# refresh-bio/LZ-ANI

Hardware: AMD Instinct MI355X
Metric: genome-pairs/sec + achieved HBM GB/s, 10k×40kbp all2all at 1/2/4/8 GPUs (higher is better)
Workload: dtype u32 (2-bit packed symbols, 64-bit lane masks; f64 only in the anchor/seed arbitration)

## Files before the change

### lz-ani_amd/csrc/lzani_kernels_pairs.h

```cpp
#pragma once

namespace lzani {

enum { SEED_BM_BITS = 14, SEED_BM_WORDS = 1 << (SEED_BM_BITS - 5), NQUEUES = 8 };
enum { AQ_CAP = 64, AQ_MAXCHUNKS = 32, AQ_LANE_CAP = 32, AQ_LDS_CAND = 128,
       SEED_PAD = 96,
       SEED_LDS_WORDS = SEED_BM_WORDS + SEED_PAD };
static_assert(2 * AQ_LDS_CAND <= SEED_BM_WORDS, "the candidate buffers of refill live in the seed bitmap");
enum : u32 { AQ_COMPLEX = 0x80000000u, AQ_LONG = 0x40000000u, AQ_POS = 0x3FFFFFFFu };
enum { AQ_NONE = 0x7FFFFFFF };

__device__ __forceinline__ u64 wballot(bool b) { return __builtin_amdgcn_ballot_w64(b); }
__device__ __forceinline__ u32 rep4(u32 b) { return __builtin_amdgcn_perm(b, b, 0u); }

#if defined(LZANI_RTC)
#define LZ_RTC_PARAMS Params{LZANI_P_MAL, LZANI_P_MSL, LZANI_P_MRD, LZANI_P_MQD, LZANI_P_REG, LZANI_P_AW, LZANI_P_AM, LZANI_P_AR}
#else
#define LZ_RTC_PARAMS Params{11, 7, 40, 40, 35, 15, 7, 3}
#endif
LZ_HD constexpr Params folded_params(int defp)
{
    return defp == 2 ? Params{15, 9, 40, 40, 60, 15, 7, 3} : defp == 9 ? LZ_RTC_PARAMS : Params{11, 7, 40, 40, 35, 15, 7, 3};
}
LZ_HD constexpr bool chain_params_ok(const Params& p)
// ... 740 lines not shown
            "ds_or_b32 %[a0], %[t]\n\t" \
            WORD("a1", "bq", K1) \
            "ds_or_b32 %[a1], %[bq]\n\t" \
            WORD("aq", "t", QK) \
            "ds_read_b32 %[aq], %[aq]\n\t" \
            "ds_write_b32 %[a0], %[zero]\n\t" \
            "ds_write_b32 %[a1], %[zero]\n\t" \
            "s_waitcnt lgkmcnt(2)\n\t" \
            "v_and_b32_e32 %[aq], %[aq], %[t]\n\t" \
            "v_cmp_ne_u32_e64 %[seed], 0, %[aq]\n\t"
#define LZ_NC_ROUND_F(WORD) LZ_NC_ROUND_X(WORD, "s_waitcnt vmcnt(0)", "qk", "rk0", "rk1")
#define LZ_NC_FTURN(WORDF, P, N, IC, IN, RN, CQ, C0, C1, NQ, N0, N1, SFX) \
            "Lnc_fturn" SFX "_%=:\n\t" \
            "s_bitcmp0_b32 %[" P "], 15\n\t" \
            "s_cbranch_scc1 Lnc_fnogo" SFX "_%=\n\t" \
            "s_bfe_u32 %[qh], %[" P "], 0x70008\n\t"         \
            "v_readlane_b32 %[" N "], %[alen], %[qh]\n\t"    \
            "v_readlane_b32 %[ap], %[apos], %[qh]\n\t" \
            "v_readlane_b32 %[bpos], %[aref], %[qh]\n\t" \
            "s_bfe_u32 %[t0], %[" N "], 0x80011\n\t" \
            "s_sub_i32 %[gap], %[ap], %[" IC "]\n\t" \
            "s_add_i32 %[" IN "], %[ap], %[t0]\n\t" \
            "s_add_i32 %[" RN "], %[bpos], %[t0]\n\t" \
            LZ_NC_LOADS_X(IN, RN, NQ, N0, N1) \
            LZ_NC_ROUND_X(WORDF, "s_waitcnt vmcnt(3)", CQ, C0, C1) \
            LZ_NC_SEEDS \
            "s_cbranch_scc1 Lnc_frec" SFX "_%=\n\t"          \
            "s_mov_b32 %[t2], %[qh]\n\t" \
            LZ_NC_COUNT
#define LZ_NC_FIX \
            "s_bfm_b64 %[m2], %[NT], 0\n\t" \
            "s_and_b64 %[seed], %[seed], %[m2]\n\t" \
            "v_cmp_gt_u32_e64 %[m2], %[NR1], %[lane]\n\t" \
            "v_cmp_gt_u32_e32 vcc, %[NT], %[lane]\n\t" \
            "s_nop 1\n\t" \
            "v_cndmask_b32_e64 %[rk1], -1, %[rk1], %[m2]\n\t" \
            "v_cndmask_b32_e32 %[qk], -1, %[qk], vcc\n\t" \
            "v_cmp_ne_u32_e32 vcc, -1, %[qk]\n\t"           \
            "s_and_b64 %[seed], %[seed], vcc\n\t" \
            "s_and_b64 %[m], %[m], vcc\n"
#define LZ_NC_SEEDS \
            "s_add_i32 %[t0], %[gap], 1\n\t" \
            "s_min_u32 %[t0], %[t0], %[NT]\n\t" \
            "s_bfm_b64 %[m], %[t0], 0\n\t" \
            "s_and_b64 %[m], %[m], %[seed]\n\t" LZ_NC_NOSEED
#define LZ_NC_COMMIT \
            "s_sub_i32 %[plit], %[t1], %[kb]\n\t"            \
            "s_sub_i32 %[prs], %[ap], %[kb]\n\t"             \
            "s_bfe_u32 %[t0], %[rec], 0x50018\n\t"           \
            "s_bfe_u32 %[lastlit], %[rec], 0x40014\n\t"      \
            "s_add_i32 %[t2], %[blen], %[t0]\n\t" \
            "s_sub_i32 %[lastb], %[t2], %[lastlit]\n\t"      \
            "s_add_i32 %[lastb], %[lastb], %[kc]\n\t" \
            "s_add_i32 %[lastlit], %[lastlit], %[kb]\n\t"    \
            "s_sub_i32 %[lastlit], %[lastlit], %[kc]\n\t" \
            "s_add_i32 %[i], %[ap], %[t2]\n\t" \
            "s_add_i32 %[rend], %[bpos], %[t2]\n\t" \
            "s_mov_b32 %[pre], %[i]\n\t" \
            "s_add_i32 %[qh], %[qh], 1\n\t" \
            LZ_NC_COUNT
        int gap, cls, fok;
        u64 m2;
        const u32* const rt2 = uniform_ptr(reinterpret_cast<const u32*>(R.t2));
        const u32* const qt2 = uniform_ptr(reinterpret_cast<const u32*>(Q.t2));
        const int qend = __builtin_amdgcn_readfirstlane((R.nfree && Q.nfree) ? iend : -(1 << 30));
        const int ocl_u = __builtin_amdgcn_readfirstlane(open_cl), oclit_u = __builtin_amdgcn_readfirstlane(open_clit);
#ifdef LZANI_CHAIN_PRIO
#define LZ_NC_PRIO_ON "s_setprio 2\n\t"
#define LZ_NC_PRIO_OFF "s_setprio 0\n\t"
#else
#define LZ_NC_PRIO_ON
#define LZ_NC_PRIO_OFF
#endif
#define LZ_NC_SPLITCHK \
            "v_readlane_b32 %[t0], %[apos], %[qh]\n\t" \
            "s_cmp_gt_i32 %[t0], %[ilim]\n\t" \
            "s_cbranch_scc1 Lnc_end_%=\n\t"
#define LZ_NC_SPLITGEN \
            "s_cmp_lg_u32 %[tnt], 0\n\t" \
            "s_cbranch_scc1 Lnc_chk_%=\n\t"
#define LZ_NC_SPLITIN , [tnt] "s"(tnt_u)
#define LZ_NC_ASM(WORD, WORDF) LZ_NC_ASM_X(WORD, WORDF, "", "", )
#define LZ_NC_ASM_X(WORD, WORDF, SPLCHK, SPLGEN, SPLIN) \
        asm volatile( \
            LZ_NC_PRIO_ON \
            "s_mov_b32 %[code], 0\n\t" \
            "s_mov_b32 %[lastb], 0\n\t" \
            "s_mov_b32 %[lastlit], 0\n\t" \
            "s_mov_b32 %[atm], 0\n\t" \
            "s_mov_b32 %[atl], 0\n\t" \
            "s_mov_b32 %[atc], 0\n\t" \
            "s_mov_b64 %[m2], -1\n\t"                       \
             \
             \
            "v_add_u32_e32 %[w1], 64, %[lane]\n\t" \
            "v_subrev_u32_e32 %[dumv], %[WIN], %[w1]\n\t" \
            "v_min_u32_e32 %[w1], %[w1], %[dumv]\n\t" \
            "v_add_u32_e32 %[dumv], %[wdum], %[lane]\n\t"   \
            "s_nop 3\n" \
            "Lnc_top_%=:\n\t" \
             \
            "s_cmp_ge_i32 %[qh], %[qc]\n\t" \
            "s_cbranch_scc1 Lnc_end_%=\n\t" \
            "v_readlane_b32 %[t0], %[apos], %[qh]\n\t" \
            "s_cmp_ge_i32 %[t0], %[i]\n\t" \
            "s_cbranch_scc1 Lnc_nodrop_%=\n\t" \
            "v_cmp_le_i32_e32 vcc, %[qh], %[lane]\n\t" \
            "v_cmp_le_i32_e64 %[m], %[i], %[apos]\n\t" \
            "s_and_b64 %[m], %[m], vcc\n\t" \
            "s_ff1_i32_b64 %[qh], %[m]\n\t" \
            "s_min_u32 %[qh], %[qh], 64\n\t" \
            "s_cmp_ge_i32 %[qh], %[qc]\n\t" \
            "s_cbranch_scc1 Lnc_end_%=\n" \
            "Lnc_nodrop_%=:\n\t" \
            "s_cmp_gt_i32 %[i], %[ilim]\n\t" \
            "s_cbranch_scc1 Lnc_end_%=\n\t" \
            "s_cmp_gt_i32 %[rend], %[rlim]\n\t" \
            "s_cbranch_scc1 Lnc_end_%=\n\t" \
            SPLCHK \
            LZ_NC_LOADS_F \
             \
             \
            "v_readlane_b32 %[blen], %[alen], %[qh]\n\t" \
            "v_readlane_b32 %[ap], %[apos], %[qh]\n\t" \
            "v_readlane_b32 %[bpos], %[aref], %[qh]\n\t" \
            "v_readlane_b32 %[rec], %[aext], %[qh]\n\t" \
            "s_mov_b32 %[t2], 0\n\t" \
            "s_mov_b32 %[cls], 0\n\t"                         \
            "s_bfe_u32 %[code], %[blen], 0x10010\n\t"        \
            "s_sext_i32_i8 %[blen], %[blen]\n\t"             \
            "s_sub_i32 %[gap], %[ap], %[i]\n\t" \
            "s_cmp_lt_i32 %[blen], 1\n\t" \
            "s_cbranch_scc1 Lnc_chk_%=\n\t" \
            "s_cmp_le_i32 %[gap], %[MQD]\n\t" \
            "s_cbranch_scc1 Lnc_close_%=\n" \
            "Lnc_distant_%=:\n\t" \
            "s_cmp_lt_i32 %[prs], 0\n\t" \
            "s_cbranch_scc1 Lnc_kept_%=\n\t" \
            "s_sub_i32 %[t1], %[pre], %[prs]\n\t" \
            "s_cmp_ge_i32 %[t1], %[REG]\n\t" \
            "s_cbranch_scc1 Lnc_kept_%=\n\t" \
            "s_sub_i32 %[t1], %[ap], %[prs]\n\t" \
            "s_add_i32 %[t1], %[t1], %[plit]\n"              \
            "Lnc_avail_%=:\n\t" \
             \
             \
            "s_cmp_eq_u32 %[code], 0\n\t" \
            "s_cbranch_scc1 Lnc_gen_%=\n\t" \
            "s_cmp_lt_i32 %[t1], %[AW]\n\t" \
            "s_cbranch_scc1 Lnc_gen_%=\n\t" \
            "s_and_b32 %[kb], %[rec], 15\n\t" \
            "s_bfe_u32 %[kc], %[rec], 0x40004\n\t" \
            "s_mov_b32 %[fok], 1\n\t" \
            "s_branch Lnc_ok_%=\n" \
            "Lnc_gen_%=:\n\t" \
            SPLGEN \
            "s_bitcmp0_b32 %[rec], 29\n\t"                   \
            "s_cbranch_scc1 Lnc_chk_%=\n\t" \
            "s_min_i32 %[t0], %[t1], %[ap]\n\t" \
            "s_min_i32 %[t0], %[t0], %[bpos]\n\t"            \
            "s_mov_b32 %[kb], 0\n\t"                           \
            "s_mov_b32 %[kc], 0\n\t" \
            "s_mov_b32 %[fok], 0\n\t" \
            "s_cmp_lt_i32 %[t0], 1\n\t" \
            "s_cbranch_scc1 Lnc_ok_%=\n\t" \
            "s_bitcmp1_b32 %[rec], 30\n\t" \
            "s_cbranch_scc1 Lnc_brkb_%=\n\t" \
            "s_min_i32 %[code], %[t0], %[AW]\n\t"            \
            "s_bfm_b32 %[code], %[code], 0\n\t"              \
            "s_and_b32 %[code], %[code], %[rec]\n\t" \
            "s_cbranch_scc1 Lnc_chk_%=\n\t" \
            "s_cmp_le_i32 %[t0], %[AW]\n\t" \
            "s_cbranch_scc1 Lnc_ok_%=\n\t" \
            "s_branch Lnc_chk_%=\n" \
            "Lnc_brkb_%=:\n\t"                                \
            "s_cmp_lt_i32 %[t0], %[AW]\n\t"                  \
            "s_cbranch_scc1 Lnc_chk_%=\n\t" \
            "s_and_b32 %[kb], %[rec], 15\n\t" \
            "s_bfe_u32 %[kc], %[rec], 0x40004\n\t" \
            "s_mov_b32 %[fok], 1\n"                           \
            "Lnc_ok_%=:\n\t" \
            "s_mov_b32 %[t2], 1\n" \
            "Lnc_chk_%=:\n\t" \
            LZ_NC_ROUND_F(WORD) \
            "s_mov_b32 %[code], 1\n\t" \
            LZ_NC_SEEDS \
            "s_cbranch_scc1 Lnc_sseed_%=\n"                  \
            "Lnc_noseed_%=:\n\t" \
            "s_cmp_lt_i32 %[blen], 1\n\t" \
            "s_cbranch_scc1 Lnc_npl_%=\n\t"                  \
            "s_mov_b32 %[code], 2\n\t" \
            "s_cmp_eq_u32 %[t2], 0\n\t" \
            "s_cbranch_scc1 Lnc_end_%=\n\t"                  \
            "s_cmp_eq_u32 %[cls], 0\n\t" \
            "s_cbranch_scc1 Lnc_commit_%=\n\t" \
             \
             \
             \
            "s_cmp_lg_u32 %[lastb], 0\n\t" \
            "s_cselect_b32 %[t0], %[lastb], %[ocl]\n\t" \
            "s_cselect_b32 %[t2], %[lastlit], %[oclit]\n\t" \
            "s_cmp_eq_u32 %[t0], 0\n\t" \
            "s_cbranch_scc1 Lnc_commit_%=\n\t" \
            "s_add_i32 %[t2], %[t2], %[t0]\n\t" \
            "s_cmp_lt_i32 %[t2], %[REG]\n\t" \
            "s_cbranch_scc1 Lnc_commit_%=\n\t" \
            "s_sub_i32 %[t2], %[t2], %[t0]\n\t" \
            "s_add_i32 %[atm], %[atm], %[t0]\n\t" \
            "s_add_i32 %[atl], %[atl], %[t2]\n\t" \
            "s_add_i32 %[atc], %[atc], 1\n" \
            "Lnc_commit_%=:\n\t" \
            LZ_NC_COMMIT \
            "s_mov_b32 %[code], 0\n\t" \
            "s_cmp_eq_u32 %[fok], 0\n\t" \
            "s_cbranch_scc1 Lnc_top_%=\n" \
             \
             \
             \
            "Lnc_fast_%=:\n\t" \
             \
             \
             \
             \
            "s_sub_i32 %[fok], %[prs], %[plit]\n\t" \
            "s_sub_i32 %[t2], %[qh], 1\n\t"                 \
            "v_readlane_b32 %[cls], %[alen], %[t2]\n"       \
            "Lnc_fstart_%=:\n\t" \
            LZ_NC_LOADS_F \
             \
             \
             \
             \
             \
            LZ_NC_FTURN(WORDF, "cls", "blen", "i", "t1", "kb", "qk", "rk0", "rk1", "qkb", "rk0b", "rk1b", "") \
            LZ_NC_FTURN(WORDF, "blen", "cls", "t1", "i", "rend", "qkb", "rk0b", "rk1b", "qk", "rk0", "rk1", "2") \
            "s_branch Lnc_fturn_%=\n" \
            "Lnc_fnogo2_%=:\n\t" \
            "s_mov_b32 %[i], %[t1]\n\t" \
            "s_mov_b32 %[rend], %[kb]\n\t" \
            "s_mov_b32 %[cls], %[blen]\n\t" \
            "s_branch Lnc_fnogo_%=\n" \
            "Lnc_frec2_%=:\n\t" \
            "s_mov_b32 %[i], %[t1]\n\t" \
            "s_mov_b32 %[rend], %[kb]\n\t" \
            "s_mov_b32 %[t0], %[cls]\n\t" \
            "s_mov_b32 %[cls], %[blen]\n\t" \
            "s_mov_b32 %[blen], %[t0]\n\t" \
            "s_waitcnt vmcnt(0)\n\t"                         \
            "v_mov_b32_e32 %[qk], %[qkb]\n\t" \
            "v_mov_b32_e32 %[rk0], %[rk0b]\n\t" \
            "v_mov_b32_e32 %[rk1], %[rk1b]\n\t" \
            "s_branch Lnc_frec_%=\n" \
             \
            "Lnc_fcont_%=:\n\t" \
            "s_bfe_u32 %[t0], %[blen], 0x80011\n\t" \
            "s_add_i32 %[i], %[ap], %[t0]\n\t" \
            "s_add_i32 %[rend], %[bpos], %[t0]\n\t" \
            "s_mov_b32 %[t2], %[qh]\n\t" \
            "s_mov_b32 %[cls], %[blen]\n\t" \
            LZ_NC_COUNT \
            "s_branch Lnc_fstart_%=\n" \
            "Lnc_fnogo_%=:\n\t"                             \
            "s_add_i32 %[qh], %[t2], 1\n" \
             \
            "Lnc_frec_%=:\n\t" \
            "v_readlane_b32 %[t0], %[apos], %[t2]\n\t" \
            "v_readlane_b32 %[t1], %[alen], %[t2]\n\t" \
            "v_readlane_b32 %[kc], %[aext], %[t2]\n\t" \
            "s_sext_i32_i8 %[t1], %[t1]\n\t" \
            "s_and_b32 %[kb], %[kc], 15\n\t" \
            "s_sub_i32 %[prs], %[t0], %[kb]\n\t" \
            "s_sub_i32 %[plit], %[t0], %[fok]\n\t" \
            "s_sub_i32 %[plit], %[plit], %[kb]\n\t" \
            "s_bfe_u32 %[lastlit], %[kc], 0x40014\n\t" \
            "s_bfe_u32 %[t0], %[kc], 0x50018\n\t" \
            "s_add_i32 %[t1], %[t1], %[t0]\n\t" \
            "s_sub_i32 %[lastb], %[t1], %[lastlit]\n\t" \
            "s_bfe_u32 %[t0], %[kc], 0x40004\n\t" \
            "s_add_i32 %[lastb], %[lastb], %[t0]\n\t" \
            "s_add_i32 %[lastlit], %[lastlit], %[kb]\n\t" \
            "s_sub_i32 %[lastlit], %[lastlit], %[t0]\n\t" \
            "s_mov_b32 %[pre], %[i]\n\t" \
            "s_bitcmp0_b32 %[cls], 15\n\t" \
            "s_cbranch_scc1 Lnc_top_%=\n"                    \
            "Lnc_fseed_%=:\n\t"                              \
            "s_mov_b32 %[code], 1\n\t" \
            LZ_NC_FIX \
            "s_cmp_eq_u64 %[m], 0\n\t"                       \
            "s_cbranch_scc1 Lnc_snone_%=\n" \
             \
             \
             \
             \
             \
             \
            "Lnc_seedev_%=:\n\t" \
            "s_ff1_i32_b64 %[t0], %[m]\n"                    \
            "Lnc_sdl_%=:\n\t" \
            "v_readlane_b32 %[t1], %[qk], %[t0]\n\t"         \
            "s_add_i32 %[t2], %[t0], %[MRD]\n\t"             \
            "s_sub_i32 %[kc], %[t2], 64\n\t" \
            "s_max_i32 %[kc], %[kc], 0\n\t" \
            "s_min_u32 %[kb], %[t2], 64\n\t" \
            "s_sub_i32 %[kb], 64, %[kb]\n\t"                 \
            "v_cmp_eq_u32_e32 vcc, %[t1], %[rk1]\n\t" \
            "s_bfm_b64 %[m2], %[kc], 0\n\t" \
            "s_and_b64 %[m2], %[m2], vcc\n\t" \
            "v_cmp_eq_u32_e32 vcc, %[t1], %[rk0]\n\t" \
            "s_bcnt1_i32_b64 %[kc], %[m2]\n\t" \
            "s_lshl_b64 vcc, vcc, %[kb]\n\t" \
            "s_bcnt1_i32_b64 %[t1], vcc\n\t" \
            "s_add_i32 %[t2], %[t1], %[kc]\n\t" \
            LZ_NC_WHY(2) \
            "s_cmp_eq_u32 %[t2], 0\n\t" \
            "s_cbranch_scc1 Lnc_sfalse_%=\n\t"               \
            "s_cmp_lg_u32 %[t2], 1\n\t" \
            "s_cbranch_scc1 Lnc_end_%=\n\t"                  \
            "s_ff1_i32_b64 %[t2], vcc\n\t" \
            "s_sub_i32 %[t2], %[t2], %[kb]\n\t" \
            "s_ff1_i32_b64 %[kc], %[m2]\n\t" \
            "s_add_i32 %[kc], %[kc], 64\n\t" \
            "s_cmp_lg_u32 %[t1], 0\n\t" \
            "s_cselect_b32 %[t2], %[t2], %[kc]\n\t"          \
            "s_add_i32 %[rec], %[rend], %[t2]\n\t"           \
            "s_add_i32 %[cls], %[i], %[t0]\n\t"              \
             \
             \
             \
             \
            LZ_NC_WHY(1) \
            "s_cmp_lg_u32 %[t0], %[gap]\n\t" \
            "s_cbranch_scc1 Lnc_snoq_%=\n\t" \
            "s_cmp_lt_i32 %[blen], 1\n\t" \
            "s_cbranch_scc1 Lnc_end_%=\n\t" \
            "s_cmp_lg_u32 %[bpos], %[rec]\n\t" \
            "s_cbranch_scc1 Lnc_end_%=\n" \
            "Lnc_snoq_%=:\n\t" \
             \
             \
             \
            "s_sub_i32 %[t1], %[qend], %[CQ64]\n\t" \
            LZ_NC_WHY(3) \
            "s_cmp_gt_i32 %[cls], %[t1]\n\t" \
            "s_cbranch_scc1 Lnc_end_%=\n\t" \
            "s_sub_i32 %[t1], %[rlim], %[C41M]\n\t" \
            "s_lshr_b32 %[t1], %[t1], 1\n\t" \
// ... 101 lines not shown
            "v_lshlrev_b32_e32 %[t], 1, %[t]\n\t" \
            "v_lshlrev_b32_e32 %[bq], 1, %[bq]\n\t" \
            "v_and_b32_e32 %[t], 30, %[t]\n\t" \
            "v_and_b32_e32 %[bq], 30, %[bq]\n\t" \
            "v_lshrrev_b32_e32 %[rk0], %[t], %[rk0]\n\t" \
            "v_lshrrev_b32_e32 %[rk1], %[bq], %[rk1]\n\t" \
            "v_xor_b32_e32 %[rk0], %[rk0], %[rk1]\n\t" \
            "v_and_b32_e32 %[rk0], 3, %[rk0]\n\t" \
            "v_cmp_eq_u32_e64 %[m], 0, %[rk0]\n\t" \
             \
            "v_add_u32_e32 %[t], %[gap], %[lane]\n\t" \
            "v_add_u32_e32 %[bq], %[kc], %[lane]\n\t" \
            "v_lshlrev_b32_e32 %[t], 1, %[t]\n\t" \
            "v_lshlrev_b32_e32 %[bq], 1, %[bq]\n\t" \
            "v_and_b32_e32 %[t], 30, %[t]\n\t" \
            "v_and_b32_e32 %[bq], 30, %[bq]\n\t" \
            "v_lshrrev_b32_e32 %[qk], %[t], %[qk]\n\t" \
            "v_lshrrev_b32_e32 %[a0], %[bq], %[a0]\n\t" \
            "v_xor_b32_e32 %[qk], %[qk], %[a0]\n\t" \
            "v_and_b32_e32 %[qk], 3, %[qk]\n\t" \
            "v_cmp_eq_u32_e64 %[m2], 0, %[qk]\n\t" \
             \
            "v_add_u32_e32 %[t], %[fok], %[lane]\n\t" \
            "v_add_u32_e32 %[bq], %[t1], %[lane]\n\t" \
            "v_lshlrev_b32_e32 %[t], 1, %[t]\n\t" \
            "v_lshlrev_b32_e32 %[bq], 1, %[bq]\n\t" \
            "v_and_b32_e32 %[t], 30, %[t]\n\t" \
            "v_and_b32_e32 %[bq], 30, %[bq]\n\t" \
            "v_lshrrev_b32_e32 %[a1], %[t], %[a1]\n\t" \
            "v_lshrrev_b32_e32 %[aq], %[bq], %[aq]\n\t" \
            "v_xor_b32_e32 %[a1], %[a1], %[aq]\n\t" \
            "v_and_b32_e32 %[a1], 3, %[a1]\n\t" \
            "v_cmp_ne_u32_e32 vcc, 0, %[a1]\n\t" \
            "s_and_b64 %[m], %[m], %[seed]\n\t"              \
            "s_and_b64 %[m2], %[m2], %[seed]\n\t"            \
            "s_mov_b64 %[seed], vcc\n\t"                     \
             \
            "s_bcnt1_i32_b64 %[t2], %[m2]\n\t" \
            "s_mov_b64 vcc, %[m]\n\t" \
            "s_nop 0\n\t" \
            "v_mbcnt_lo_u32_b32 %[t], vcc_lo, 0\n\t" \
            "v_mbcnt_hi_u32_b32 %[t], vcc_hi, %[t]\n\t" \
            "s_mov_b64 vcc, %[m2]\n\t" \
            "s_nop 0\n\t" \
            "v_mbcnt_lo_u32_b32 %[bq], vcc_lo, 0\n\t" \
            "v_mbcnt_hi_u32_b32 %[bq], vcc_hi, %[bq]\n\t" \
            "v_add_u32_e32 %[t], %[t2], %[t]\n\t" \
            "v_sub_u32_e32 %[t], %[t], %[bq]\n\t" \
            "v_cmp_ge_u32_e32 vcc, %[kb], %[lane]\n\t" \
            "s_nop 1\n\t" \
            "v_cndmask_b32_e32 %[t], 0, %[t], vcc\n\t"       \
            "s_nop 1\n\t" \
            "v_max_u32_dpp %[t], %[t], %[t] row_shr:1 row_mask:0xf bank_mask:0xf bound_ctrl:0\n\t" \
            "s_nop 1\n\t" \
            "v_max_u32_dpp %[t], %[t], %[t] row_shr:2 row_mask:0xf bank_mask:0xf bound_ctrl:0\n\t" \
            "s_nop 1\n\t" \
            "v_max_u32_dpp %[t], %[t], %[t] row_shr:4 row_mask:0xf bank_mask:0xf bound_ctrl:0\n\t" \
            "s_nop 1\n\t" \
            "v_max_u32_dpp %[t], %[t], %[t] row_shr:8 row_mask:0xf bank_mask:0xf bound_ctrl:0\n\t" \
            "s_nop 1\n\t" \
            "v_max_u32_dpp %[t], %[t], %[t] row_bcast:15 row_mask:0xa bank_mask:0xf\n\t" \
            "s_nop 1\n\t" \
            "v_max_u32_dpp %[t], %[t], %[t] row_bcast:31 row_mask:0xc bank_mask:0xf\n\t" \
            "s_nop 1\n\t" \
            "v_readlane_b32 %[t2], %[t], 63\n\t"             \
             \
             \
             \
            "s_mov_b64 vcc, %[seed]\n\t" \
            "s_lshl_b32 %[gap], vcc_lo, %[AW1]\n\t" \
            "s_lshr_b32 %[kb], vcc_lo, %[AW1C]\n\t" \
            "s_lshl_b32 %[kc], vcc_hi, %[AW1]\n\t" \
            "s_or_b32 %[kc], %[kc], %[kb]\n\t" \
            "s_lshr_b32 %[kb], vcc_hi, %[AW1C]\n\t" \
            "v_mov_b32_e32 %[rk0], %[gap]\n\t" \
            "v_mov_b32_e32 %[rk1], %[kc]\n\t" \
            "v_mov_b32_e32 %[qk], %[kb]\n\t" \
            "v_cmp_gt_u32_e32 vcc, 32, %[lane]\n\t" \
            "v_alignbit_b32 %[a0], %[rk1], %[rk0], %[lane]\n\t" \
            "v_alignbit_b32 %[a1], %[qk], %[rk1], %[lane]\n\t" \
            "v_cndmask_b32_e32 %[a0], %[a1], %[a0], vcc\n\t" \
            "v_and_b32_e32 %[a0], %[AWM], %[a0]\n\t" \
            "v_bcnt_u32_b32 %[a1], %[a0], 0\n\t" \
            "v_and_b32_e32 %[a0], %[ARM], %[a0]\n\t" \
            "v_cmp_lt_u32_e32 vcc, %[AM], %[a1]\n\t"             \
            "v_cmp_eq_u32_e64 %[m], 0, %[a0]\n\t"            \
            "s_nop 0\n\t" \
            "s_cmp_eq_u64 vcc, 0\n\t" \
            "s_cbranch_scc1 Lnc_end_%=\n\t"                  \
            "s_ff1_i32_b64 %[kb], vcc\n\t" \
            "s_cmp_ge_u32 %[kb], 63\n\t" \
            "s_cbranch_scc1 Lnc_end_%=\n\t" \
            "s_add_i32 %[kb], %[kb], 1\n\t" \
            "s_bfm_b64 %[m2], %[kb], 0\n\t" \
            "s_and_b64 %[m], %[m], %[m2]\n\t"                \
            "s_mov_b32 %[kb], 0\n\t"                          \
            "s_mov_b32 %[kc], 0\n\t"                          \
            "s_cbranch_scc0 Lnc_sext_%=\n\t" \
            "s_flbit_i32_b64 %[kb], %[m]\n\t" \
            "s_sub_i32 %[kb], 64, %[kb]\n\t"                 \
            "s_bfm_b64 %[m2], %[kb], 0\n\t" \
            "s_and_b64 %[m2], %[m2], %[seed]\n\t" \
            "s_bcnt1_i32_b64 %[kc], %[m2]\n"                  \
            "Lnc_sext_%=:\n\t" \
             \
            "s_cmp_lg_u32 %[lastb], 0\n\t" \
            "s_cselect_b32 %[gap], %[lastb], %[ocl]\n\t" \
            "s_cselect_b32 %[rec], %[lastlit], %[oclit]\n\t" \
            "s_add_i32 %[gap], %[gap], %[t2]\n\t"            \
            "s_add_i32 %[gap], %[gap], %[blen]\n\t" \
            "s_add_i32 %[gap], %[gap], %[kb]\n\t" \
            "s_sub_i32 %[lastb], %[gap], %[kc]\n\t"          \
            "s_add_i32 %[rec], %[rec], %[t0]\n\t" \
            "s_sub_i32 %[rec], %[rec], %[t2]\n\t" \
            "s_add_i32 %[lastlit], %[rec], %[kc]\n\t"        \
            "s_add_i32 %[i], %[t1], %[kb]\n\t" \
            "s_add_i32 %[rend], %[fok], %[kb]\n\t" \
            "s_mov_b32 %[pre], %[i]\n\t" \
            "s_mov_b32 %[code], 0\n\t" \
            "s_mov_b64 %[m2], -1\n\t" \
            LZ_NC_COUNT \
            "s_branch Lnc_top_%=\n" \
             \
             \
            "Lnc_sfalse_%=:\n\t" \
            "s_bitset0_b64 %[m], %[t0]\n\t" \
            "s_cmp_eq_u64 %[m], 0\n\t" \
            "s_cbranch_scc1 Lnc_snone_%=\n\t" \
            "s_ff1_i32_b64 %[t0], %[m]\n\t" \
            "s_branch Lnc_sdl_%=\n" \
            "Lnc_snone_%=:\n\t" \
            "s_mov_b32 %[code], 0\n\t" \
            "s_mov_b64 %[m2], -1\n\t" \
            "s_bitcmp1_b32 %[cls], 15\n\t" \
            "s_cbranch_scc1 Lnc_fcont_%=\n\t" \
            "s_mov_b64 %[m2], 0\n\t" \
            "s_branch Lnc_top_%=\n" \
            "Lnc_sseed_%=:\n\t"                             \
            "s_cmp_eq_u64 %[m2], 0\n\t" \
            "s_mov_b64 %[m2], -1\n\t" \
            "s_cbranch_scc1 Lnc_noseed_%=\n\t" \
            "s_branch Lnc_fseed_%=\n" \
            "Lnc_kept_%=:\n\t"                               \
            "s_mov_b32 %[cls], 1\n\t"                         \
            "s_mov_b32 %[t1], %[gap]\n\t" \
            "s_branch Lnc_avail_%=\n" \
            "Lnc_close_%=:\n\t"                              \
            "s_add_i32 %[t1], %[rend], %[gap]\n\t" \
            "s_sub_i32 %[t1], %[bpos], %[t1]\n\t" \
            "s_abs_i32 %[t1], %[t1]\n\t" \
            "s_cmp_le_i32 %[t1], %[MRD]\n\t" \
            "s_cbranch_scc1 Lnc_chk_%=\n\t" \
            "s_branch Lnc_distant_%=\n" \
            "Lnc_npl_%=:\n\t" \
            LZ_NC_FIX \
            "Lnc_end_%=:\n\t" \
            "s_waitcnt vmcnt(0) lgkmcnt(0)\n\t" \
            LZ_NC_PRIO_OFF \
            "s_nop 4" \
            : LZ_NC_COUNT_OPERAND [i] "+s"(i), [rend] "+s"(r_end), [qh] "+s"(qh), [prs] "+s"(prev_rs), [pre] "+s"(prev_re), [plit] "+s"(pre_lit), \
              [code] "=&s"(code), [ap] "=&s"(ap), [bpos] "=&s"(bpos), [blen] "=&s"(blen), [lastb] "=&s"(last_cl), [lastlit] "=&s"(last_clit), [rec] "=&s"(rec), \
              [t0] "=&s"(t0), [t1] "=&s"(t1), [t2] "=&s"(t2), [kb] "=&s"(kb), [kc] "=&s"(kc), [m] "=&s"(m), [seed] "=&s"(seed), \
              [gap] "=&s"(gap), [cls] "=&s"(cls), [fok] "=&s"(fok), [atm] "=&s"(add_tm), [atl] "=&s"(add_tl), [atc] "=&s"(add_tc), [m2] "=&s"(m2), \
              [rk0] "=&v"(rk0), [rk1] "=&v"(rk1), [qk] "=&v"(qk), [a0] "=&v"(a0), [a1] "=&v"(a1), [aq] "=&v"(aq), [t] "=&v"(t), [bq] "=&v"(bq), [w1] "=&v"(w1), [dumv] "=&v"(dumv), [qkb] "=&v"(qkb), [rk0b] "=&v"(rk0b), [rk1b] "=&v"(rk1b) \
            : [qc] "s"(qc_u), [ilim] "s"(ilim_u), [rlim] "s"(rlim_u), [qks] "s"(qks), [rks] "s"(rks), [ocl] "s"(ocl_u), [oclit] "s"(oclit_u), \
              [rt2] "s"(rt2), [qt2] "s"(qt2), [qend] "s"(qend), [wdum] "s"((int)SEED_BM_WORDS) SPLIN, \
              [apos] "v"(a_pos), [alen] "v"(a_len), [aref] "v"(a_ref), [aext] "v"(a_ext), [lane] "v"(lane), \
              [ldsb] "v"(ldsb), [zero] "v"(zero), [one] "v"(one), \
              [MQD] "n"(MQD), [MRD] "n"(MRD), [REG] "n"(REG), [AW] "n"(AW), [NT] "n"(NT), [WIN] "s"((int)WIN), [NR1] "n"(WIN - 64), [MSL] "n"(MSL), [MSL64] "n"(MSL + 64), [C41M] "n"(3 * MRD + 1 - WIN - MSL), [C40M] "n"(MRD - MSL), [CQ64] "n"(MRD + 64), [C2MRD] "n"(2 * MRD), \
              [AW1] "n"(AW - 1), [AW1C] "n"(33 - AW), [AWM] "n"((1 << AW) - 1), [ARM] "n"(((1 << AR) - 1) << (AW - AR)), [AM] "n"(AM), [KS5] "n"(2 * MSL + 5), [KS] "n"(2 * MSL) \
            : "vcc", "scc", "memory");
#ifdef LZANI_PHASE_TIME
        const unsigned long long pt_t0 = pt_now();
#endif
        if constexpr (SPLITW) {
            if constexpr (MSL == 9) { LZ_NC_ASM_X(LZ_NC_WORD9, LZ_NC_WORD9, LZ_NC_SPLITCHK, LZ_NC_SPLITGEN, LZ_NC_SPLITIN) }
            else if constexpr (MSL == 8) { LZ_NC_ASM_X(LZ_NC_WORD8, LZ_NC_WORD8, LZ_NC_SPLITCHK, LZ_NC_SPLITGEN, LZ_NC_SPLITIN) }
            else if constexpr (CP::NF) { LZ_NC_ASM_X(LZ_NC_WORD7, LZ_NC_WORD7N, LZ_NC_SPLITCHK, LZ_NC_SPLITGEN, LZ_NC_SPLITIN) }
            else { LZ_NC_ASM_X(LZ_NC_WORD7, LZ_NC_WORD7, LZ_NC_SPLITCHK, LZ_NC_SPLITGEN, LZ_NC_SPLITIN) }
        } else
        if constexpr (MSL == 9) { LZ_NC_ASM(LZ_NC_WORD9, LZ_NC_WORD9) }
        else if constexpr (MSL == 8) { LZ_NC_ASM(LZ_NC_WORD8, LZ_NC_WORD8) }
        else if constexpr (CP::NF) { LZ_NC_ASM(LZ_NC_WORD7, LZ_NC_WORD7N) }
        else { LZ_NC_ASM(LZ_NC_WORD7, LZ_NC_WORD7) }
#ifdef LZANI_PHASE_TIME
        pt_chain += pt_now() - pt_t0;
#endif
        q_head = qh;
        if constexpr (JOIN) {
            if (code == 0 && scan_pos >= i && scan_pos < iend && (qh >= q_cnt || (i > ilim_q && restart_at != i))) refill_only = true;
        }
        pre_round = code == 1;
        if (code == 0) LZ_PS(16); else if (code == 1) LZ_PS(17); else if (code == 2) LZ_PS(18); else LZ_PS(19);
        pre_seed = seed; pre_rk0 = rk0; pre_rk1 = rk1; pre_qk = qk;
        if (code == 2) { adv = ap - i; last_src = q_head++; }
        if (code == 4) { adv = ap; last_src = -1; }
#ifdef LZANI_CHAIN_STATS
        st[0] += 1; st[1] += ncnt; st[2] += code == 0; st[3] += code == 1 && seed != 0; st[4] += code == 1 && seed == 0; st[5] += code == 2;
        if (code == 2) {
            const int g2 = ap - i;
            const bool close = g2 <= MQD && iabs(bpos - (r_end + g2)) <= MRD;
            const bool kept = prev_rs < 0 || prev_re - prev_rs >= REG;
            const bool nofwd = !((u32)rec & EXT_REC_FWDK);
            sr[0] += close; sr[1] += !close && kept; sr[2] += !close && !kept && nofwd; sr[3] += !close && !kept && !nofwd;
        }
        if (code == 1 && seed != 0) {
            sw[0] += why == 1; sw[2] += why == 2; sw[3] += why == 3; sw[4] += why == 4; sw[5] += why == 0;
        }
        if (code == 4) sw[6] += 1;
#endif
        return code;
    }

    static constexpr bool HAS_STRETCH_CHAIN = CHAIN != 0 && (ChainP<CHAIN>::MQD <= ChainP<CHAIN>::MRD) &&
                                              (!JOIN || ChainP<CHAIN>::MAL >= 13 || LZANI_STRETCH_DENSE);
    __device__ __forceinline__ int stretch_chain(int& i, int& r_end, int& cl, int& clit, int& kind, u64& Bf, int& adv, u32& hqa)
    {
        typedef ChainP<CHAIN> CP;
        enum { MQD = CP::MQD, MRD = CP::MRD, MSL = CP::MSL, AW = CP::AW, AM = CP::AM, AR = CP::AR, NT = CP::NT, WIN = CP::WIN };
        const int ilim = SPLITW ? imin(iend - NT, stop_i - (int)SPLIT_MARGIN) : iend - NT, rlim = R.len - MSL + 1 - WIN;
        const u32 ldsb = (u32)(size_t)bitmap;
        const u32 zero = 0, one = 1;
        const u32* const qks = uniform_ptr(qkS);
        const u32* const rks = uniform_ptr(rkS);
        const u32* const qkl = uniform_ptr(qkL);
        const u32* const rt2 = uniform_ptr(reinterpret_cast<const u32*>(R.t2));
        const u32* const qt2 = uniform_ptr(reinterpret_cast<const u32*>(Q.t2));
        const u32* const twp = uniform_ptr(I.tw);
        const u32* const bkp = uniform_ptr(I.bk);
        const int qend = __builtin_amdgcn_readfirstlane((R.nfree && Q.nfree) ? iend : -(1 << 30));
        const int tbits = __builtin_amdgcn_readfirstlane(I.kb - I.dirbits), pbits = __builtin_amdgcn_readfirstlane(I.posbits);
        const u32 tagm = (u32)__builtin_amdgcn_readfirstlane((int)I.tagmask);
        int ncm, t0, t1, t2, kb, kc, gap, rec, cls, fok, blen, anc, aent;
        u64 m, seed, m2, pmk;
        u32 rk0, rk1, qk, hq, a0, a1, aq, t, bq, w1, dumv;
        [[maybe_unused]] u64 cwa, cwb;
        [[maybe_unused]] u32 e0, e1, e2, e3, tagl;
        [[maybe_unused]] const unsigned long long* const cbp = JOIN ? reinterpret_cast<const unsigned long long*>(uniform_ptr(reinterpret_cast<const u32*>(cand_bits))) : nullptr;
#if defined(LZANI_STAMPS) || defined(LZANI_PATH_STATS)
        constexpr bool unify = true;
#else
        constexpr bool unify = SPLITW;
#endif
        int ilim_u = ilim, rlim_u = rlim;
        if constexpr (unify) {
            i = __builtin_amdgcn_readfirstlane(i); r_end = __builtin_amdgcn_readfirstlane(r_end);
            cl = __builtin_amdgcn_readfirstlane(cl); clit = __builtin_amdgcn_readfirstlane(clit);
            ilim_u = __builtin_amdgcn_readfirstlane(ilim); rlim_u = __builtin_amdgcn_readfirstlane(rlim);
        }
#ifdef LZANI_PATH_STATS
        int why = 0;
#define LZ_SC_WHY(n) "s_mov_b32 %[why], " #n "\n\t"
#define LZ_SC_WHY_OPERAND [why] "=&s"(why),
#else
#define LZ_SC_WHY(n)
#define LZ_SC_WHY_OPERAND
#endif
#define LZ_SC_P_CANDLOAD
#define LZ_SC_P_TWADDR \
            "v_lshrrev_b32_e32 %[bq], %[TB], %[hq]\n\t"      \
            "v_cmp_ge_u32_e32 vcc, %[t0], %[lane]\n\t"
#define LZ_SC_P_TWADDR2 \
            "v_lshlrev_b32_e32 %[bq], 2, %[bq]\n\t" \
            "v_cndmask_b32_e32 %[bq], 0, %[bq], vcc\n\t"
#define LZ_SC_P_TWLOAD \
            "s_mov_b64 %[pmk], vcc\n\t" \
            "s_nop 0\n\t" \
            "global_load_dword %[bq], %[bq], %[twp]\n\t"
#define LZ_SC_P_VWAIT "s_waitcnt vmcnt(0)\n\t"
#define LZ_SC_P_TWSWAR \
            "v_and_b32_e32 %[a0], %[TAGM], %[hq]\n\t" \
            "v_or_b32_e32 %[a0], 0x80, %[a0]\n\t" \
            "v_perm_b32 %[a0], %[a0], %[a0], %[zero]\n\t" \
            "v_xor_b32_e32 %[a0], %[a0], %[bq]\n\t"          \
            "v_subrev_u32_e32 %[a1], 0x01010101, %[a0]\n\t" \
            "v_not_b32_e32 %[a0], %[a0]\n\t" \
            "v_and_b32_e32 %[a1], %[a1], %[a0]\n\t" \
            "v_and_b32_e32 %[a1], 0x80808080, %[a1]\n\t"
#define LZ_SC_P_CANDMASK \
            "v_cmp_ne_u32_e32 vcc, 0, %[a1]\n\t" \
            "s_mov_b64 %[m2], vcc\n\t" \
            "v_cmp_eq_u32_e32 vcc, 0x808080ff, %[bq]\n\t"    \
            "s_or_b64 %[m2], %[m2], vcc\n\t" \
            "s_and_b64 %[m2], %[m2], %[pmk]\n\t"
#define LZ_SC_P_ANCENTRY \
             \
            "v_readlane_b32 %[kc], %[a1], %[t0]\n\t"         \
            "v_readlane_b32 %[t1], %[bq], %[t0]\n\t"         \
            "v_readlane_b32 %[t2], %[hq], %[t0]\n\t" \
            "s_cmp_eq_u32 %[t1], 0x808080ff\n\t" \
            LZ_SC_WHY(7) "s_cbranch_scc1 Lsc_end_%=\n\t" \
            "s_sub_u32 %[t1], %[kc], 1\n\t" \
            "s_and_b32 %[t1], %[t1], %[kc]\n\t" \
            "s_cmp_lg_u32 %[t1], 0\n\t" \
            "s_cbranch_scc1 Lsc_end_%=\n\t"                  \
            "s_ff1_i32_b32 %[kc], %[kc]\n\t" \
            "s_lshr_b32 %[kc], %[kc], 3\n\t"                 \
            "s_lshr_b32 %[t2], %[t2], %[TB]\n\t" \
            "s_lshl_b32 %[t2], %[t2], 2\n\t" \
            "s_add_u32 %[t2], %[t2], %[kc]\n\t" \
            "s_lshl_b32 %[t2], %[t2], 2\n\t" \
            "s_load_dword %[aent], %[bkp], %[t2]\n\t" \
            "s_mov_b32 %[anc], 1\n"
#define LZ_SC_P_ANCCHECK \
            "s_bfm_b32 %[anc], %[PB], 0\n\t" \
            "s_and_b32 %[aent], %[aent], %[anc]\n\t" \
// ... 898 lines not shown
```

Measured before the change: 15.78 million.

## Resolve forward anchor extension inline in the scalar chain loop instead of exiting

Adds a forward-extension path inside the inline-asm chaining loop. When a match ends and the bit-29 flag is set (t2=2), the loop loads the next 64 packed symbols from reference and query and computes mismatch masks with ballot plus alignbit windowing. It then scores the anchor window and commits the extended match, continuing the loop rather than returning to the outer code. This avoids leaving and re-entering the kernel loop for common continuation cases, but adds global loads, a vmcnt wait and extra branches to the hot loop, along with more scalar register pressure.

```diff
diff --git a/lz-ani_amd/csrc/lzani_kernels_pairs.h b/lz-ani_amd/csrc/lzani_kernels_pairs.h
--- a/lz-ani_amd/csrc/lzani_kernels_pairs.h
+++ b/lz-ani_amd/csrc/lzani_kernels_pairs.h
@@ -916,11 +916,10 @@
             "s_and_b32 %[kb], %[rec], 15\n\t" \
             "s_bfe_u32 %[kc], %[rec], 0x40004\n\t" \
             "s_mov_b32 %[fok], 1\n\t" \
-            "s_branch Lnc_ok_%=\n" \
+            "s_mov_b32 %[t2], 1\n\t" \
+            "s_branch Lnc_chk_%=\n" \
             "Lnc_gen_%=:\n\t" \
             SPLGEN \
-            "s_bitcmp0_b32 %[rec], 29\n\t"                   \
-            "s_cbranch_scc1 Lnc_chk_%=\n\t" \
             "s_min_i32 %[t0], %[t1], %[ap]\n\t" \
             "s_min_i32 %[t0], %[t0], %[bpos]\n\t"            \
             "s_mov_b32 %[kb], 0\n\t"                           \
@@ -943,8 +942,9 @@
             "s_and_b32 %[kb], %[rec], 15\n\t" \
             "s_bfe_u32 %[kc], %[rec], 0x40004\n\t" \
             "s_mov_b32 %[fok], 1\n"                           \
-            "Lnc_ok_%=:\n\t" \
-            "s_mov_b32 %[t2], 1\n" \
+            "Lnc_ok_%=:\n\t"                                  \
+            "s_bitcmp1_b32 %[rec], 29\n\t"                   \
+            "s_cselect_b32 %[t2], 1, 2\n"                    \
             "Lnc_chk_%=:\n\t" \
             LZ_NC_ROUND_F(WORD) \
             "s_mov_b32 %[code], 1\n\t" \
@@ -954,8 +954,8 @@
             "s_cmp_lt_i32 %[blen], 1\n\t" \
             "s_cbranch_scc1 Lnc_npl_%=\n\t"                  \
             "s_mov_b32 %[code], 2\n\t" \
-            "s_cmp_eq_u32 %[t2], 0\n\t" \
-            "s_cbranch_scc1 Lnc_end_%=\n\t"                  \
+            "s_cmp_lg_u32 %[t2], 1\n\t" \
+            "s_cbranch_scc1 Lnc_fwd_%=\n\t"                  \
             "s_cmp_eq_u32 %[cls], 0\n\t" \
             "s_cbranch_scc1 Lnc_commit_%=\n\t" \
              \
@@ -1363,6 +1363,121 @@
             "s_cmp_le_i32 %[t1], %[MRD]\n\t" \
             "s_cbranch_scc1 Lnc_chk_%=\n\t" \
             "s_branch Lnc_distant_%=\n" \
+             \
+             \
+             \
+             \
+             \
+             \
+            "Lnc_fwd_%=:\n\t" \
+            "s_cmp_eq_u32 %[t2], 0\n\t" \
+            "s_cbranch_scc1 Lnc_end_%=\n\t" \
+            "s_add_i32 %[t0], %[ap], %[blen]\n\t"            \
+            "s_add_i32 %[t2], %[t0], 64\n\t" \
+            "s_sub_i32 %[gap], %[qend], %[C40M]\n\t"         \
+            "s_cmp_gt_i32 %[t2], %[gap]\n\t" \
+            "s_cbranch_scc1 Lnc_end_%=\n\t" \
+            "s_add_i32 %[fok], %[bpos], %[blen]\n\t"         \
+            "s_add_i32 %[t2], %[fok], 64\n\t" \
+            "s_sub_i32 %[gap], %[rlim], %[C41M]\n\t" \
+            "s_lshr_b32 %[gap], %[gap], 1\n\t"               \
+            "s_cmp_le_i32 %[t2], %[gap]\n\t" \
+            "s_cbranch_scc1 Lnc_fwdin_%=\n\t" \
+            "s_add_i32 vcc_lo, %[gap], %[C2MRD]\n\t"         \
+            "s_cmp_lt_i32 %[fok], vcc_lo\n\t" \
+            "s_cbranch_scc1 Lnc_end_%=\n\t" \
+            "s_add_i32 vcc_lo, vcc_lo, %[gap]\n\t" \
+            "s_cmp_gt_i32 %[t2], vcc_lo\n\t" \
+            "s_cbranch_scc1 Lnc_end_%=\n" \
+            "Lnc_fwdin_%=:\n\t" \
+            "v_add_u32_e32 %[a1], %[fok], %[lane]\n\t" \
+            "v_add_u32_e32 %[aq], %[t0], %[lane]\n\t" \
+            "v_lshrrev_b32_e32 %[a1], 4, %[a1]\n\t" \
+            "v_lshrrev_b32_e32 %[aq], 4, %[aq]\n\t" \
+            "v_lshlrev_b32_e32 %[a1], 2, %[a1]\n\t" \
+            "v_lshlrev_b32_e32 %[aq], 2, %[aq]\n\t" \
+            "s_nop 0\n\t" \
+            "global_load_dword %[a1], %[a1], %[rt2]\n\t" \
+            "global_load_dword %[aq], %[aq], %[qt2]\n\t" \
+            "v_add_u32_e32 %[t], %[fok], %[lane]\n\t" \
+            "v_add_u32_e32 %[bq], %[t0], %[lane]\n\t" \
+            "v_lshlrev_b32_e32 %[t], 1, %[t]\n\t" \
+            "v_lshlrev_b32_e32 %[bq], 1, %[bq]\n\t" \
+            "v_and_b32_e32 %[t], 30, %[t]\n\t" \
+            "v_and_b32_e32 %[bq], 30, %[bq]\n\t" \
+            "s_waitcnt vmcnt(0)\n\t" \
+            "v_lshrrev_b32_e32 %[a1], %[t], %[a1]\n\t" \
+            "v_lshrrev_b32_e32 %[aq], %[bq], %[aq]\n\t" \
+            "v_xor_b32_e32 %[a1], %[a1], %[aq]\n\t" \
+            "v_and_b32_e32 %[a1], 3, %[a1]\n\t" \
+            "v_cmp_ne_u32_e32 vcc, 0, %[a1]\n\t" \
+            "s_nop 1\n\t" \
+            "s_mov_b64 %[m2], vcc\n\t"                       \
+            "s_lshl_b32 %[gap], vcc_lo, %[AW1]\n\t"          \
+            "s_lshr_b32 %[t2], vcc_lo, %[AW1C]\n\t" \
+            "s_lshl_b32 %[t0], vcc_hi, %[AW1]\n\t" \
+            "s_or_b32 %[t0], %[t0], %[t2]\n\t" \
+            "s_lshr_b32 %[t2], vcc_hi, %[AW1C]\n\t" \
+            "v_mov_b32_e32 %[a0], %[gap]\n\t" \
+            "v_mov_b32_e32 %[t], %[t0]\n\t" \
+            "v_mov_b32_e32 %[bq], %[t2]\n\t" \
+            "v_cmp_gt_u32_e32 vcc, 32, %[lane]\n\t" \
+            "v_alignbit_b32 %[a1], %[t], %[a0], %[lane]\n\t" \
+            "v_alignbit_b32 %[aq], %[bq], %[t], %[lane]\n\t" \
+            "v_cndmask_b32_e32 %[a1], %[aq], %[a1], vcc\n\t" \
+            "v_and_b32_e32 %[a1], %[AWM], %[a1]\n\t" \
+            "v_bcnt_u32_b32 %[aq], %[a1], 0\n\t" \
+            "v_and_b32_e32 %[a1], %[ARM], %[a1]\n\t" \
+            "v_cmp_lt_u32_e32 vcc, %[AM], %[aq]\n\t"         \
+            "v_cmp_eq_u32_e64 %[m], 0, %[a1]\n\t"            \
+            "s_nop 0\n\t" \
+            "s_cmp_eq_u64 vcc, 0\n\t" \
+            "s_cbranch_scc1 Lnc_end_%=\n\t"                  \
+            "s_ff1_i32_b64 %[t2], vcc\n\t" \
+            "s_cmp_ge_u32 %[t2], 63\n\t" \
+            "s_cbranch_scc1 Lnc_end_%=\n\t" \
+            "s_add_i32 %[t2], %[t2], 1\n\t" \
+            "s_bfm_b64 vcc, %[t2], 0\n\t" \
+            "s_and_b64 %[m], %[m], vcc\n\t"                  \
+            "s_mov_b32 %[gap], 0\n\t"                        \
+            "s_mov_b32 %[fok], 0\n\t"                        \
+            "s_cbranch_scc0 Lnc_fwdc_%=\n\t" \
+            "s_flbit_i32_b64 %[gap], %[m]\n\t" \
+            "s_sub_i32 %[gap], 64, %[gap]\n\t"               \
+            "s_bfm_b64 vcc, %[gap], 0\n\t" \
+            "s_and_b64 vcc, vcc, %[m2]\n\t" \
+            "s_bcnt1_i32_b64 %[fok], vcc\n"                  \
+            "Lnc_fwdc_%=:\n\t"                               \
+            "s_cmp_eq_u32 %[cls], 0\n\t" \
+            "s_cbranch_scc1 Lnc_fwdm_%=\n\t" \
+            "s_cmp_lg_u32 %[lastb], 0\n\t" \
+            "s_cselect_b32 %[t0], %[lastb], %[ocl]\n\t" \
+            "s_cselect_b32 %[t2], %[lastlit], %[oclit]\n\t" \
+            "s_cmp_eq_u32 %[t0], 0\n\t" \
+            "s_cbranch_scc1 Lnc_fwdm_%=\n\t" \
+            "s_add_i32 %[t2], %[t2], %[t0]\n\t" \
+            "s_cmp_lt_i32 %[t2], %[REG]\n\t" \
+            "s_cbranch_scc1 Lnc_fwdm_%=\n\t" \
+            "s_sub_i32 %[t2], %[t2], %[t0]\n\t" \
+            "s_add_i32 %[atm], %[atm], %[t0]\n\t" \
+            "s_add_i32 %[atl], %[atl], %[t2]\n\t" \
+            "s_add_i32 %[atc], %[atc], 1\n" \
+            "Lnc_fwdm_%=:\n\t"                               \
+            "s_sub_i32 %[plit], %[t1], %[kb]\n\t" \
+            "s_sub_i32 %[prs], %[ap], %[kb]\n\t" \
+            "s_add_i32 %[t2], %[blen], %[gap]\n\t" \
+            "s_sub_i32 %[lastb], %[t2], %[fok]\n\t" \
+            "s_add_i32 %[lastb], %[lastb], %[kc]\n\t" \
+            "s_add_i32 %[lastlit], %[fok], %[kb]\n\t" \
+            "s_sub_i32 %[lastlit], %[lastlit], %[kc]\n\t" \
+            "s_add_i32 %[i], %[ap], %[t2]\n\t" \
+            "s_add_i32 %[rend], %[bpos], %[t2]\n\t" \
+            "s_mov_b32 %[pre], %[i]\n\t" \
+            "s_add_i32 %[qh], %[qh], 1\n\t" \
+            LZ_NC_COUNT \
+            "s_mov_b32 %[code], 0\n\t" \
+            "s_mov_b64 %[m2], -1\n\t" \
+            "s_branch Lnc_top_%=\n" \
             "Lnc_npl_%=:\n\t" \
             LZ_NC_FIX \
             "Lnc_end_%=:\n\t" \
```

After: 15.96 million, median of 6. +1.2%, better.
